# ynotstartups/implisolid

Measured on AMD Instinct MI355X. Metric: Mvoxels/s (eval+MC) at 256^3 & 512^3, higher is better.
Workload: dtype f32; 1 GPU; config4: seeded ~20-node MP5 CSG tree with twist/union/difference (scenes.config4, seed 20251015), box [-1,1]^3, R=512, eval+MC, mesh resident in HBM; resolution=512, voxels=134217728, samples=135005697, cells=135796744, verts=360248, faces=720496, program_instr=42, tree_depth=8, parallelism=zslab1, voxels_per_rank=134217728

## Files before the change

### implisolid_amd/csrc/mc.hip

```cpp
#include <algorithm>
#include <cstdlib>
#include <stdexcept>

#include "eval_bricks.hpp"
#include "ifunc_device.hpp"
#include "kernels.hpp"
#include "mc_device.hpp"
#include "batch_device.hpp"

namespace impli {

GridDesc make_grid(int R, const float box[6], int cz0, int cz1, int cz_emit) {
    GridDesc g{};
    g.R = R;
    g.res = R + 5;
    g.n = R + 3;
    g.m = R + 2;
    for (int a = 0; a < 3; ++a) {
        const float width = box[2 * a + 1] - box[2 * a];
        g.w[a] = width / (float)R;
        g.lo[a] = box[2 * a];
        g.i0[a] = box[2 * a] / g.w[a] - 2.f;
    }
    g.cz0 = cz0;
    g.cz1 = cz1;
    g.cz_emit = cz_emit;
    g.fz0 = cz0;
    g.fz1 = cz1 + 1;
    g.n_cells = (int64_t)g.m * g.m * (cz1 - cz0);
    return g;
}

void build_case_table(CaseInfo out[256]) {
    for (int ci = 0; ci < 256; ++ci) {
        CaseInfo c{};
        const char* s = IMPLI_MC_TRI_CASES[ci];
        int n = 0;
        for (; s[n]; ++n) c.tri[n] = (uint8_t)((s[n] <= '9') ? s[n] - '0' : s[n] - 'a' + 10);
        c.ntri = (uint8_t)(n / 3);
        c.rank[0] = c.rank[1] = c.rank[2] = -1;
        int r = 0;
        for (int k = 0; k < n; ++k) {
            const int e = c.tri[k];
            const int slot = (e == 5) ? 0 : (e == 6) ? 1 : (e == 10) ? 2 : -1;
            if (slot >= 0 && c.rank[slot] < 0) c.rank[slot] = (int8_t)r++;
        }
        c.nown = (uint8_t)r;
        static const int owner_of_edge[12] = {5, 4, 4, 6, 2, 0, 0, 1, 3, 2, 0, 1};
        for (int k = 0; k < n; ++k) c.owners = (uint8_t)(c.owners | (1u << owner_of_edge[c.tri[k]]));
        auto neg = [ci](int k) { return (ci >> k) & 1; };
        const int crossing = (neg(5) ^ neg(6)) + (neg(6) ^ neg(7)) + (neg(2) ^ neg(6));
        int ec = 0, ei = 0, v = 0, ff = 0, opp = 0;
        for (const auto& e : kCubeEdges) { ec += neg(e[0]) ^ neg(e[1]); ei += neg(e[0]) & neg(e[1]); }
        for (int k = 0; k < 8; ++k) v += neg(k);
        for (const auto& f : kCubeFaces) ff += neg(f[0]) & neg(f[1]) & neg(f[2]) & neg(f[3]);
        for (const auto& o : kCubeOpposite) opp += (v == 6 && !neg(o[0]) && !neg(o[1])) ? 1 : 0;
        const int ntri_formula = (ci == 0 || ci == 255) ? 0 : ec - 2 * (v - ei + ff + 2 * opp);
        if (crossing != c.nown || (c.ntri > 0) != (ci != 0 && ci != 255) || ntri_formula != c.ntri)
            throw std::runtime_error("marching cubes: case table violates the count kernel's assumptions");
        out[ci] = c;
    }
}

namespace {

__device__ __forceinline__ uint32_t wave_sum(uint32_t x) {
#pragma unroll
    for (int o = 32; o > 0; o >>= 1) x += __shfl_xor(x, o, 64);
    return x;
}

template <int BS>
__device__ __forceinline__ void mc_count_body(const GridDesc& g, const MCBuffers& b) {
    static_assert(BS % 64 == 0 && BS >= kGroupUnits, "whole waves; wave 0 takes a lane per unit of the group");
    __shared__ uint32_t s_u[kGroupUnits][4];
    __shared__ uint32_t s_cm[kGroupUnits];
    __shared__ uint16_t s_fp[kGroupUnits * kMaxChunks];
    __shared__ uint32_t s_nf;
    const int t = threadIdx.x;
    const int64_t G = blockIdx.x;
    const int nch = n_chunks(g), npairs = kGroupUnits * nch;
    const int64_t rows = n_rows(g), nu = n_units(g);
    const int64_t row0 = G * kGroupUnits * kUnitRows;
    int ui[2], ch[2];
    bool in[2];
    uint32_t mk[2];
    auto marks = [&](int p0) {
#pragma unroll
        for (int q = 0; q < 2; ++q) {
            const int p = p0 + q * BS + t;
            ui[q] = p / nch;
            ch[q] = p - ui[q] * nch;
            in[q] = p < npairs && G * kGroupUnits + ui[q] < nu;
            mk[q] = b.mark_id;
        }
        if (b.umark) {
#pragma unroll
            for (int q = 0; q < 2; ++q) mk[q] = b.umark[in[q] ? (G * kGroupUnits + ui[q]) * nch + ch[q] : 0];
        }
    };
    marks(0);
    for (int k = t; k < 4 * kGroupUnits; k += BS) (&s_u[0][0])[k] = 0u;
    for (int k = t; k < kGroupUnits; k += BS) s_cm[k] = 0u;
    if (t == 0) s_nf = 0u;
    __syncthreads();
    for (int p0 = 0;;) {
        const bool c0 = in[0] & (mk[0] == b.mark_id), c1 = in[1] & (mk[1] == b.mark_id);
        const uint64_t m0 = __ballot(c0), m1 = __ballot(c1);
        const uint32_t n0 = (uint32_t)__popcll((unsigned long long)m0), n1 = (uint32_t)__popcll((unsigned long long)m1);
        const uint64_t below = (1ull << (t & 63)) - 1ull;
        uint32_t base = 0;
        if ((t & 63) == 0 && n0 + n1) base = atomicAdd(&s_nf, n0 + n1);
        base = __shfl(base, 0, 64);
        if (c0) s_fp[base + __popcll((unsigned long long)(m0 & below))] = (uint16_t)(ui[0] * kMaxChunks + ch[0]);
        if (c1) s_fp[base + n0 + __popcll((unsigned long long)(m1 & below))] = (uint16_t)(ui[1] * kMaxChunks + ch[1]);
        p0 += 2 * BS;
        if (p0 >= npairs) break;
        marks(p0);
    }
    __syncthreads();
    const int n_items = (int)s_nf * kUnitRows;
    for (int i = t; i < n_items; i += BS) {
        ChunkBits k;
        const uint32_t pr = s_fp[i / kUnitRows];
        const int ui = (int)(pr / kMaxChunks), c = (int)(pr % kMaxChunks);
        const int rb = ui * kUnitRows + i % kUnitRows;
        const bool ok = row0 + rb < rows;
        load_chunk(g, b.signs, ok ? row0 + rb : 0, c, k);
        if (!ok) k.nt = 0;
        if (!k.nt) continue;
        if (c < kChunkMaskBits) atomicOr(&s_cm[ui], 1u << c);
        const unsigned own = (unsigned)(__popcll((unsigned long long)((k.t01 ^ k.t11) & k.nt)) +
                                        __popcll((unsigned long long)((k.s11 ^ k.t11) & k.nt)) +
                                        __popcll((unsigned long long)((k.t10 ^ k.t11) & k.nt)));
        unsigned tri = 0, act = 0, hal = 0;
        if (k.z >= g.cz_emit) {
            act = (unsigned)__popcll((unsigned long long)k.nt);
            tri = chunk_triangles(k);
        } else {
            hal = own;
        }
        uint32_t* d = s_u[ui];
        if (own) atomicAdd(&d[0], own);
        if (tri) atomicAdd(&d[1], tri);
        atomicAdd(&d[2], act | ((uint32_t)__popcll((unsigned long long)k.nt) << 16));
        if (hal) atomicAdd(&d[3], hal);
    }
    __syncthreads();
    if (t < 64) {
        const int64_t u = G * kGroupUnits + t;
        const uint32_t own = s_u[t][0], tri = s_u[t][1], act = s_u[t][2] & 0xffffu, ntc = s_u[t][2] >> 16, hal = s_u[t][3];
        const bool ne = u < nu && (own | tri) != 0;
        const uint32_t eo = wave_incl_scan<uint32_t>(own, t) - own;
        const uint32_t et = wave_incl_scan<uint32_t>(tri, t) - tri;
        const uint32_t ea = wave_incl_scan<uint32_t>(act, t) - act;
        const uint64_t m = __ballot(ne);
        const uint32_t pos = (uint32_t)__popcll((unsigned long long)(m & ((1ull << t) - 1ull)));
        const uint32_t parts = ne ? min((uint32_t)kMaxParts, max(1u, (act + kPartCells - 1) / kPartCells)) : 0u;
        const bool heavy = act > kHeavyCells;
        const bool small = ne && ntc <= kPairCells && nch <= kChunkMaskBits &&
                           (uint32_t)(kUnitRows * __popc(s_cm[t])) <= kPairCells;
        const uint32_t ph = heavy ? parts : 0u, pl = (heavy || small) ? 0u : parts, ps = small ? 1u : 0u;
        const uint32_t eph = wave_incl_scan<uint32_t>(ph, t) - ph, epl = wave_incl_scan<uint32_t>(pl, t) - pl;
        const uint64_t msm = __ballot(small);
        const uint32_t eps = (uint32_t)__popcll((unsigned long long)(msm & ((1ull << t) - 1ull)));
        if (ne) {
            b.unit_cnt[G * kGroupUnits + pos] = make_uint4((uint32_t)t, eo, et, ea);
            b.unit_part[G * kGroupUnits + pos] =
                (heavy ? eph : small ? eps : epl) | (parts << 16) | ((uint32_t)heavy << 20) | (ps << 21);
            b.unit_cmask[G * kGroupUnits + pos] = s_cm[t];
        }
        const uint32_t sums[kScanParts + 1] = {__shfl(eo + own, 63, 64), __shfl(et + tri, 63, 64),
                                               __shfl(ea + act, 63, 64), wave_sum(hal), __shfl(eph + ph, 63, 64),
                                               __shfl(epl + pl, 63, 64), (uint32_t)__popcll((unsigned long long)msm),
                                               (uint32_t)__popcll((unsigned long long)m)};
        if (t <= kScanParts) {
            const uint32_t v = t == 0 ? sums[0] : t == 1 ? sums[1] : t == 2 ? sums[2] : t == 3 ? sums[3]
                             : t == 4 ? sums[4] : t == 5 ? sums[5] : t == 6 ? sums[6] : sums[7];
            b.scan_blk[(int64_t)t * gridDim.x + G] = v;
        }
    }
}
__global__ __launch_bounds__(512) void k_mc_count(GridDesc g, MCBuffers b) { mc_count_body<512>(g, b); }
__global__ __launch_bounds__(256) void k_mc_count_s(GridDesc g, MCBuffers b) { mc_count_body<256>(g, b); }

constexpr int kScanBlock = 256;
constexpr int kScanRows = kScanParts + 1;
template <int BS = kScanBlock>
__device__ __forceinline__ void unit_scan_body(const GridDesc& g, const MCBuffers& b) {
    static_assert(BS >= kGroupUnits, "a lane per unit of the group");
    __shared__ uint32_t s_part[BS / 64][kScanRows];
    __shared__ uint32_t s_base[kScanRows];
    const int64_t G = blockIdx.x, ng = n_groups(g);
    const int t = threadIdx.x, lane = t & 63, wid = t >> 6;
    const bool last = G == ng - 1;
    const uint32_t nne = b.scan_blk[kScanParts * ng + G];
    if (nne == 0 && !last) return;
    const uint4 e = b.unit_cnt[G * kGroupUnits + (t < (int)nne ? t : 0)];
    const uint32_t pp = b.unit_part[G * kGroupUnits + (t < (int)nne ? t : 0)];
    const uint32_t cm = b.unit_cmask[G * kGroupUnits + (t < (int)nne ? t : 0)];
    uint32_t acc[kScanRows] = {0u, 0u, 0u, 0u, 0u, 0u, 0u, 0u};
#pragma unroll 4
    for (int64_t i = t; i < G; i += BS)
#pragma unroll
        for (int c = 0; c < kScanRows; ++c) acc[c] += b.scan_blk[c * ng + i];
#pragma unroll
    for (int c = 0; c < kScanRows; ++c) {
        const uint32_t s = wave_sum(acc[c]);
        if (lane == 0) s_part[wid][c] = s;
    }
    __syncthreads();
    if (t < kScanRows) {
        uint32_t s = 0;
#pragma unroll
        for (int w = 0; w < BS / 64; ++w) s += s_part[w][t];
        s_base[t] = s;
    }
    __syncthreads();
    if (t < (int)nne) {
        const uint4 ent = make_uint4((uint32_t)(G * kGroupUnits) + e.x, s_base[0] + e.y, s_base[1] + e.z, s_base[2] + e.w);
        const uint32_t P = (pp >> 16) & 15u;
        const bool heavy = (pp >> 20) & 1u, small = (pp >> 21) & 1u;
        const uint32_t r = (heavy ? s_base[4] : small ? s_base[6] : s_base[5]) + (pp & 0xffffu);
        for (uint32_t q = 0; q < P; ++q) {
            const uint32_t at = heavy ? r + q : b.cap_parts - (small ? 2u : 1u) - 2u * (r + q);
            b.ulist[at] = ent;
            b.upart[at] = q | (P << 4) | (cm << 8);
        }
    }
    if (last && t == 0) {
        const uint32_t nh = s_base[4] + b.scan_blk[4 * ng + G];
        const uint32_t ns = s_base[6] + b.scan_blk[6 * ng + G];
        b.counters[7] = nh;
        b.counters[8] = ns;
        b.counters[0] = nh + (ns + 1u) / 2u + s_base[5] + b.scan_blk[5 * ng + G];
        b.counters[1] = s_base[3] + b.scan_blk[3 * ng + G];
        b.counters[2] = s_base[0] + b.scan_blk[G];
        b.counters[3] = s_base[1] + b.scan_blk[ng + G];
        b.counters[4] = s_base[2] + b.scan_blk[2 * ng + G];
        b.counters[5] = s_base[3] + b.scan_blk[3 * ng + G];
        b.counters[6] = s_base[7] + nne;
    }
}
__global__ __launch_bounds__(kScanBlock) void k_unit_scan(GridDesc g, MCBuffers b) { unit_scan_body<>(g, b); }

__global__ __launch_bounds__(64 * kVertsWaves) __attribute__((amdgpu_waves_per_eu(6))) void k_mc_cells(const CaseInfo* __restrict__ cases, GridDesc g, MCBuffers b) {
    mc_cells_body(cases, g, b);
}

constexpr unsigned kFacesBlocks = 2048;
static_assert(kFacesBlocks % 8 == 0, "k_mc_faces' XCD remap needs a multiple of 8 blocks");

__constant__ uint8_t c_edge_owner_idx[12] = {5, 4, 4, 6, 2, 0, 0, 1, 3, 2, 0, 1};
__constant__ uint8_t c_edge_slot[12] = {1, 0, 1, 0, 1, 0, 1, 0, 2, 2, 2, 2};

__device__ __forceinline__ void face_record(const CaseInfo* s_case, uint32_t (*s_w)[256], const GridDesc& g,
                                            const MCBuffers& b, uint32_t Voff, uint32_t i) {
    const int t = threadIdx.x;
    const uint4 r = b.records[i];
    const uint32_t L = r.x, ci = r.y, fbase = r.z;
    const CaseInfo& C = s_case[ci];
    const int ntri = C.ntri;
    if (fbase + ntri > (uint64_t)b.cap_f) { *b.overflow = 1u; return; }
    const uint32_t need = C.owners;
    const uint32_t m = (uint32_t)g.m, m2 = m * m;
    const uint32_t d[6] = {1u, m, m + 1u, m2, m2 + m, m2 + 1u};
    const IdTriple* vid = reinterpret_cast<const IdTriple*>(b.vid);
    IdTriple w[7];
    w[0] = vid[L];
#pragma unroll
    for (int q = 0; q < 6; ++q) w[q + 1] = vid[((need >> (q + 1)) & 1u) ? L - d[q] : L];
#pragma unroll
    for (int e = 0; e < 12; ++e) {
        const IdTriple& q = w[c_edge_owner_idx[e]];
        const int sl = c_edge_slot[e];
        s_w[e][t] = sl == 0 ? q.a : sl == 1 ? q.b : q.c;
    }
    int32_t* out = b.faces + 3 * (size_t)fbase;
    for (int k = 0; k < ntri; ++k) {
        IdTriple f;
        f.a = Voff + s_w[C.tri[3 * k]][t];
        f.b = Voff + s_w[C.tri[3 * k + 1]][t];
        f.c = Voff + s_w[C.tri[3 * k + 2]][t];
        *reinterpret_cast<IdTriple*>(out + 3 * k) = f;
    }
}

__device__ __forceinline__ void mc_faces_body(const CaseInfo* __restrict__ cases, const GridDesc& g, const MCBuffers& b) {
    __shared__ CaseInfo s_case[256];
    __shared__ uint32_t s_w[12][256];
    const int t = threadIdx.x;
    s_case[t] = cases[t];
    __syncthreads();
    const uint32_t n_rec = b.counters[4];
    const uint32_t lim = n_rec < (uint64_t)b.cap_rec ? n_rec : (uint32_t)b.cap_rec;
    uint32_t Voff = b.offsets ? b.offsets[0] : 0u;
    if (b.gathered)
        for (int r = 0; r < b.rank; ++r) Voff += b.gathered[4 * r] - b.gathered[4 * r + 3];
    const uint32_t nb = gridDim.x, lb = (blockIdx.x % 8u) * (nb / 8u) + blockIdx.x / 8u;
    const uint32_t per = (lim + nb - 1u) / nb, i_end = min(lim, (lb + 1u) * per);
    for (uint32_t i = lb * per + t; i < i_end; i += 256) face_record(s_case, s_w, g, b, Voff, i);
}

__global__ __launch_bounds__(256) void k_mc_faces(const CaseInfo* __restrict__ cases, GridDesc g, MCBuffers b) {
    mc_faces_body(cases, g, b);
}

constexpr int kBatchCountLanes = 128;
__global__ __launch_bounds__(kBatchCountLanes) void k_mc_count_b(const ObjArgs* __restrict__ objs, GridDesc g) {
    mc_count_body<kBatchCountLanes>(g, objs[blockIdx.y].mc);
}
template <int B>
__global__ __launch_bounds__(B) void k_unit_scan_b(const ObjArgs* __restrict__ objs, GridDesc g) {
    unit_scan_body<B>(g, objs[blockIdx.y].mc);
}
__global__ __launch_bounds__(64 * kVertsWaves) void k_mc_cells_b(const CaseInfo* __restrict__ cases,
                                                                const ObjArgs* __restrict__ objs, int n, GridDesc g) {
    __shared__ uint32_t s_cw[256];
    __shared__ uint64_t s_bits[kVertsWaves][9][64];
    __shared__ uint32_t s_excl[kVertsWaves][64];
    __shared__ uint32_t s_pre[kMaxBatchObjects + 4];
    const int t = threadIdx.x, wid = t >> 6;
    for (int k = t; k < 256; k += blockDim.x) s_cw[k] = case_word(cases[k]);
    const uint32_t total = batch_prefix(objs, n, 0, 1u, 0xffffffffu, s_pre);
    for (uint32_t e = blockIdx.x * kVertsWaves + wid; e < total; e += gridDim.x * kVertsWaves) {
        const int k = __builtin_amdgcn_readfirstlane(batch_object_of(s_pre, n, e));
        mc_cells_item(s_cw, g, objs[k].mc, e - s_pre[k], s_bits[wid], s_excl[wid]);
    }
}
__global__ __launch_bounds__(256) void k_gather_counters(const ObjArgs* __restrict__ objs, int n, uint32_t* __restrict__ out) {
    const int i = blockIdx.x * 256 + threadIdx.x;
    if (i < n * kCounterWords) out[i] = objs[i / kCounterWords].counters[i % kCounterWords];
}
__global__ __launch_bounds__(256) void k_zero_pieces(const ZeroPiece* __restrict__ pieces) {
    const ZeroPiece z = pieces[blockIdx.x];
    uint8_t* p = reinterpret_cast<uint8_t*>(z.p);
    const uint32_t n16 = z.n / 16;
    for (uint32_t i = threadIdx.x; i < n16; i += 256) reinterpret_cast<uint4*>(p)[i] = uint4{0, 0, 0, 0};
    for (uint32_t i = n16 * 16 + threadIdx.x; i < z.n; i += 256) p[i] = 0;
}
__global__ __launch_bounds__(256) void k_mc_faces_b(const CaseInfo* __restrict__ cases, const ObjArgs* __restrict__ objs,
                                                    int n, GridDesc g) {
    __shared__ CaseInfo s_case[256];
    __shared__ uint32_t s_w[12][256];
    __shared__ uint32_t s_pre[kMaxBatchObjects + 4];
    const int t = threadIdx.x;
    s_case[t] = cases[t];
    const uint32_t total = batch_prefix(objs, n, 4, 1u, 0xffffffffu, s_pre);
    for (uint32_t gi = blockIdx.x * 256 + t; gi < total; gi += gridDim.x * 256) {
        const int k = batch_object_of(s_pre, n, gi);
        const MCBuffers& b = objs[k].mc;
        const uint32_t i = gi - s_pre[k];
        if (i >= (uint64_t)b.cap_rec) { *b.overflow = 1u; continue; }
        face_record(s_case, s_w, g, b, b.offsets ? b.offsets[0] : 0u, i);
    }
}

}

void launch_mc_count(const CaseInfo* d_cases, const GridDesc& g, const MCBuffers& b, hipStream_t s) {
    const int64_t ng = n_groups(g);
    if (ng == 0) return;
    (void)d_cases;
    if (n_chunks(g) == 1) k_mc_count_s<<<(unsigned)ng, 256, 0, s>>>(g, b);
    else k_mc_count<<<(unsigned)ng, 512, 0, s>>>(g, b);
}

void launch_mc_scan(const GridDesc& g, const MCBuffers& b, hipStream_t s) {
    const int64_t ng = n_groups(g);
    if (ng > 0) k_unit_scan<<<(unsigned)ng, kScanBlock, 0, s>>>(g, b);
}

void launch_mc_faces(const CaseInfo* d_cases, const GridDesc& g, const MCBuffers& b, hipStream_t s) {
    k_mc_faces<<<kFacesBlocks, 256, 0, s>>>(d_cases, g, b);
}

void launch_mc_verts(const CaseInfo* d_cases, const GridDesc& g, const MCBuffers& b, hipStream_t s) {
    const int64_t nu = n_units(g);
    if (nu > 0) {
        k_mc_cells<<<(unsigned)std::min<int64_t>((nu + kVertsWaves - 1) / kVertsWaves, kVertsMaxBlocks),
                     64 * kVertsWaves, 0, s>>>(d_cases, g, b);
    }
}

}

namespace impli {

constexpr unsigned kBatchCellBlocks = 4096, kBatchFaceBlocks = 2048;

void launch_gather_counters(const ObjArgs* d_objs, int n, uint32_t* d_out, hipStream_t s) {
    if (n > 0) k_gather_counters<<<(unsigned)((n * kCounterWords + 255) / 256), 256, 0, s>>>(d_objs, n, d_out);
}

void launch_zero_pieces(const ZeroPiece* d_pieces, int n, hipStream_t s) {
    if (n > 0) k_zero_pieces<<<(unsigned)n, 256, 0, s>>>(d_pieces);
}

void launch_batch_mc(const ObjArgs* d_objs, int n, const CaseInfo* d_cases, const GridDesc& g, hipStream_t s) {
    const int64_t ng = n_groups(g), nu = n_units(g);
    if (ng == 0 || n <= 0) return;
    k_mc_count_b<<<dim3((unsigned)ng, (unsigned)n), kBatchCountLanes, 0, s>>>(d_objs, g);
    if (ng <= 64) k_unit_scan_b<64><<<dim3((unsigned)ng, (unsigned)n), 64, 0, s>>>(d_objs, g);
    else k_unit_scan_b<kScanBlock><<<dim3((unsigned)ng, (unsigned)n), kScanBlock, 0, s>>>(d_objs, g);
    (void)nu;
    k_mc_cells_b<<<kBatchCellBlocks, 64 * kVertsWaves, 0, s>>>(d_cases, d_objs, n, g);
    k_mc_faces_b<<<kBatchFaceBlocks, 256, 0, s>>>(d_cases, d_objs, n, g);
}

}
```

Measured before the change: 1.438 million Mvoxels/s.

## Batch scan loads with DPP reductions and pack face case tables into shared memory

The unit scan kernel now issues several iterations of scan_blk loads before accumulating, replaces the shuffle-based wave sum with a DPP row reduction plus readlane, drops one block barrier and the s_base stage, and reads the group's own sums through lanes 0-7. The faces kernel packs each case's triangle edge indices into a 64-bit nibble word and its owners/ntri into one word in shared memory, and prefetches the next record before each face_record call. The scan kernels also get a waves-per-EU hint. The aim is to cut latency in the scan and shared-memory traffic in the faces kernel, at the cost of more code complexity and possible register pressure.

```diff
diff --git a/implisolid_amd/csrc/mc.hip b/implisolid_amd/csrc/mc.hip
--- a/implisolid_amd/csrc/mc.hip
+++ b/implisolid_amd/csrc/mc.hip
@@ -186,63 +186,92 @@
 
 constexpr int kScanBlock = 256;
 constexpr int kScanRows = kScanParts + 1;
+constexpr int kScanAhead = 4;
+__device__ __forceinline__ uint32_t wave_total_dpp(uint32_t x) {
+    x += (uint32_t)__builtin_amdgcn_update_dpp(0, (int)x, 0x111, 0xf, 0xf, false);
+    x += (uint32_t)__builtin_amdgcn_update_dpp(0, (int)x, 0x112, 0xf, 0xf, false);
+    x += (uint32_t)__builtin_amdgcn_update_dpp(0, (int)x, 0x114, 0xf, 0xf, false);
+    x += (uint32_t)__builtin_amdgcn_update_dpp(0, (int)x, 0x118, 0xf, 0xf, false);
+    x += (uint32_t)__builtin_amdgcn_update_dpp(0, (int)x, 0x142, 0xa, 0xf, false);
+    x += (uint32_t)__builtin_amdgcn_update_dpp(0, (int)x, 0x143, 0xc, 0xf, false);
+    return (uint32_t)__builtin_amdgcn_readlane((int)x, 63);
+}
+__device__ __forceinline__ uint32_t load_at(const uint32_t* p, uint32_t i) {
+    return *reinterpret_cast<const uint32_t*>(reinterpret_cast<const char*>(p) + (i << 2));
+}
 template <int BS = kScanBlock>
 __device__ __forceinline__ void unit_scan_body(const GridDesc& g, const MCBuffers& b) {
-    static_assert(BS >= kGroupUnits, "a lane per unit of the group");
-    __shared__ uint32_t s_part[BS / 64][kScanRows];
-    __shared__ uint32_t s_base[kScanRows];
-    const int64_t G = blockIdx.x, ng = n_groups(g);
-    const int t = threadIdx.x, lane = t & 63, wid = t >> 6;
-    const bool last = G == ng - 1;
-    const uint32_t nne = b.scan_blk[kScanParts * ng + G];
-    if (nne == 0 && !last) return;
-    const uint4 e = b.unit_cnt[G * kGroupUnits + (t < (int)nne ? t : 0)];
-    const uint32_t pp = b.unit_part[G * kGroupUnits + (t < (int)nne ? t : 0)];
-    const uint32_t cm = b.unit_cmask[G * kGroupUnits + (t < (int)nne ? t : 0)];
+    static_assert(BS >= kGroupUnits && BS % 64 == 0, "a lane per unit of the group, whole waves");
+    static_assert(kScanRows == 8, "lanes 0-7 of a wave hold the group's own sums");
+    constexpr int W = BS / 64;
+    __shared__ uint32_t s_part[kScanRows][W];
+    const uint32_t G = blockIdx.x, ng = (uint32_t)n_groups(g);
+    const uint32_t t = threadIdx.x, lane = t & 63u, wid = t >> 6;
+    const bool last = G == ng - 1u;
+    const uint32_t mine = b.scan_blk[(lane & 7u) * ng + G];
+    const uint32_t slot = G * kGroupUnits + (t & (uint32_t)(kGroupUnits - 1));
+    const uint4 e = b.unit_cnt[slot];
+    const uint32_t pp = b.unit_part[slot];
+    const uint32_t cm = b.unit_cmask[slot];
     uint32_t acc[kScanRows] = {0u, 0u, 0u, 0u, 0u, 0u, 0u, 0u};
-#pragma unroll 4
-    for (int64_t i = t; i < G; i += BS)
-#pragma unroll
-        for (int c = 0; c < kScanRows; ++c) acc[c] += b.scan_blk[c * ng + i];
-#pragma unroll
-    for (int c = 0; c < kScanRows; ++c) {
-        const uint32_t s = wave_sum(acc[c]);
-        if (lane == 0) s_part[wid][c] = s;
-    }
+    for (uint32_t i0 = 0; i0 < G; i0 += kScanAhead * BS) {
+        uint32_t v[kScanAhead][kScanRows];
+#pragma unroll
+        for (int q = 0; q < kScanAhead; ++q) {
+            const uint32_t i = i0 + q * BS + t;
+#pragma unroll
+            for (int c = 0; c < kScanRows; ++c) v[q][c] = load_at(b.scan_blk + c * ng, i < G ? i : 0u);
+        }
+#pragma unroll
+        for (int q = 0; q < kScanAhead; ++q)
+#pragma unroll
+            for (int c = 0; c < kScanRows; ++c) acc[c] += i0 + q * BS + t < G ? v[q][c] : 0u;
+    }
+    uint32_t tot[kScanRows];
+#pragma unroll
+    for (int c = 0; c < kScanRows; ++c) tot[c] = wave_total_dpp(acc[c]);
+    if (lane == 0) {
+#pragma unroll
+        for (int c = 0; c < kScanRows; ++c) s_part[c][wid] = tot[c];
+    }
+    const uint32_t nne = (uint32_t)__builtin_amdgcn_readlane((int)mine, kScanParts);
     __syncthreads();
-    if (t < kScanRows) {
+    auto base = [&](int c) {
         uint32_t s = 0;
 #pragma unroll
-        for (int w = 0; w < BS / 64; ++w) s += s_part[w][t];
-        s_base[t] = s;
-    }
-    __syncthreads();
-    if (t < (int)nne) {
-        const uint4 ent = make_uint4((uint32_t)(G * kGroupUnits) + e.x, s_base[0] + e.y, s_base[1] + e.z, s_base[2] + e.w);
+        for (int w = 0; w < W; ++w) s += s_part[c][w];
+        return s;
+    };
+    if (t < nne) {
+        const uint4 ent = make_uint4(G * kGroupUnits + e.x, base(0) + e.y, base(1) + e.z, base(2) + e.w);
         const uint32_t P = (pp >> 16) & 15u;
         const bool heavy = (pp >> 20) & 1u, small = (pp >> 21) & 1u;
-        const uint32_t r = (heavy ? s_base[4] : small ? s_base[6] : s_base[5]) + (pp & 0xffffu);
+        const uint32_t r = base(heavy ? 4 : small ? 6 : 5) + (pp & 0xffffu);
         for (uint32_t q = 0; q < P; ++q) {
             const uint32_t at = heavy ? r + q : b.cap_parts - (small ? 2u : 1u) - 2u * (r + q);
             b.ulist[at] = ent;
             b.upart[at] = q | (P << 4) | (cm << 8);
         }
     }
-    if (last && t == 0) {
-        const uint32_t nh = s_base[4] + b.scan_blk[4 * ng + G];
-        const uint32_t ns = s_base[6] + b.scan_blk[6 * ng + G];
-        b.counters[7] = nh;
-        b.counters[8] = ns;
-        b.counters[0] = nh + (ns + 1u) / 2u + s_base[5] + b.scan_blk[5 * ng + G];
-        b.counters[1] = s_base[3] + b.scan_blk[3 * ng + G];
-        b.counters[2] = s_base[0] + b.scan_blk[G];
-        b.counters[3] = s_base[1] + b.scan_blk[ng + G];
-        b.counters[4] = s_base[2] + b.scan_blk[2 * ng + G];
-        b.counters[5] = s_base[3] + b.scan_blk[3 * ng + G];
-        b.counters[6] = s_base[7] + nne;
-    }
-}
-__global__ __launch_bounds__(kScanBlock) void k_unit_scan(GridDesc g, MCBuffers b) { unit_scan_body<>(g, b); }
+    if (last && t < 64u) {
+        const uint32_t total = base((int)(lane & 7u)) + mine;
+        uint32_t T[kScanRows];
+#pragma unroll
+        for (int c = 0; c < kScanRows; ++c) T[c] = (uint32_t)__builtin_amdgcn_readlane((int)total, c);
+        if (t == 0) {
+            b.counters[7] = T[4];
+            b.counters[8] = T[6];
+            b.counters[0] = T[4] + (T[6] + 1u) / 2u + T[5];
+            b.counters[1] = T[3];
+            b.counters[2] = T[0];
+            b.counters[3] = T[1];
+            b.counters[4] = T[2];
+            b.counters[5] = T[3];
+            b.counters[6] = T[7];
+        }
+    }
+}
+__global__ __launch_bounds__(kScanBlock) __attribute__((amdgpu_waves_per_eu(8))) void k_unit_scan(GridDesc g, MCBuffers b) { unit_scan_body<>(g, b); }
 
 __global__ __launch_bounds__(64 * kVertsWaves) __attribute__((amdgpu_waves_per_eu(6))) void k_mc_cells(const CaseInfo* __restrict__ cases, GridDesc g, MCBuffers b) {
     mc_cells_body(cases, g, b);
@@ -254,15 +283,26 @@
 __constant__ uint8_t c_edge_owner_idx[12] = {5, 4, 4, 6, 2, 0, 0, 1, 3, 2, 0, 1};
 __constant__ uint8_t c_edge_slot[12] = {1, 0, 1, 0, 1, 0, 1, 0, 2, 2, 2, 2};
 
-__device__ __forceinline__ void face_record(const CaseInfo* s_case, uint32_t (*s_w)[256], const GridDesc& g,
-                                            const MCBuffers& b, uint32_t Voff, uint32_t i) {
+struct FaceCases {
+    uint64_t tri[256];
+    uint32_t ow[256];
+};
+__device__ __forceinline__ void face_case_store(FaceCases& fc, int ci, const CaseInfo& c) {
+    uint64_t tri = 0;
+#pragma unroll
+    for (int k = 0; k < 15; ++k) tri |= (uint64_t)(c.tri[k] & 15u) << (4 * k);
+    fc.tri[ci] = tri;
+    fc.ow[ci] = (uint32_t)c.owners | ((uint32_t)c.ntri << 8);
+}
+__device__ __forceinline__ void face_record(const FaceCases& fc, uint32_t (*s_w)[256], const GridDesc& g,
+                                            const MCBuffers& b, uint32_t Voff, const uint4 r) {
     const int t = threadIdx.x;
-    const uint4 r = b.records[i];
     const uint32_t L = r.x, ci = r.y, fbase = r.z;
-    const CaseInfo& C = s_case[ci];
-    const int ntri = C.ntri;
+    const uint32_t ow = fc.ow[ci];
+    uint64_t tri = fc.tri[ci];
+    const int ntri = (int)(ow >> 8);
     if (fbase + ntri > (uint64_t)b.cap_f) { *b.overflow = 1u; return; }
-    const uint32_t need = C.owners;
+    const uint32_t need = ow & 0xffu;
     const uint32_t m = (uint32_t)g.m, m2 = m * m;
     const uint32_t d[6] = {1u, m, m + 1u, m2, m2 + m, m2 + 1u};
     const IdTriple* vid = reinterpret_cast<const IdTriple*>(b.vid);
@@ -277,29 +317,37 @@
         s_w[e][t] = sl == 0 ? q.a : sl == 1 ? q.b : q.c;
     }
     int32_t* out = b.faces + 3 * (size_t)fbase;
-    for (int k = 0; k < ntri; ++k) {
+    for (int k = 0; k < ntri; ++k, tri >>= 12) {
         IdTriple f;
-        f.a = Voff + s_w[C.tri[3 * k]][t];
-        f.b = Voff + s_w[C.tri[3 * k + 1]][t];
-        f.c = Voff + s_w[C.tri[3 * k + 2]][t];
+        f.a = Voff + s_w[(uint32_t)tri & 15u][t];
+        f.b = Voff + s_w[((uint32_t)tri >> 4) & 15u][t];
+        f.c = Voff + s_w[((uint32_t)tri >> 8) & 15u][t];
         *reinterpret_cast<IdTriple*>(out + 3 * k) = f;
     }
 }
 
 __device__ __forceinline__ void mc_faces_body(const CaseInfo* __restrict__ cases, const GridDesc& g, const MCBuffers& b) {
-    __shared__ CaseInfo s_case[256];
+    __shared__ FaceCases s_fc;
     __shared__ uint32_t s_w[12][256];
     const int t = threadIdx.x;
-    s_case[t] = cases[t];
-    __syncthreads();
+    const CaseInfo c = cases[t];
     const uint32_t n_rec = b.counters[4];
-    const uint32_t lim = n_rec < (uint64_t)b.cap_rec ? n_rec : (uint32_t)b.cap_rec;
     uint32_t Voff = b.offsets ? b.offsets[0] : 0u;
     if (b.gathered)
         for (int r = 0; r < b.rank; ++r) Voff += b.gathered[4 * r] - b.gathered[4 * r + 3];
+    const uint32_t lim = n_rec < (uint64_t)b.cap_rec ? n_rec : (uint32_t)b.cap_rec;
     const uint32_t nb = gridDim.x, lb = (blockIdx.x % 8u) * (nb / 8u) + blockIdx.x / 8u;
     const uint32_t per = (lim + nb - 1u) / nb, i_end = min(lim, (lb + 1u) * per);
-    for (uint32_t i = lb * per + t; i < i_end; i += 256) face_record(s_case, s_w, g, b, Voff, i);
+    const uint32_t first = lb * per;
+    uint32_t i = first + t;
+    uint4 r = *(first < i_end ? b.records + (i < i_end ? i : first) : reinterpret_cast<const uint4*>(cases));
+    face_case_store(s_fc, t, c);
+    __syncthreads();
+    while (i < i_end) {
+        face_record(s_fc, s_w, g, b, Voff, r);
+        i += 256;
+        if (i < i_end) r = b.records[i];
+    }
 }
 
 __global__ __launch_bounds__(256) void k_mc_faces(const CaseInfo* __restrict__ cases, GridDesc g, MCBuffers b) {
@@ -311,7 +359,7 @@
     mc_count_body<kBatchCountLanes>(g, objs[blockIdx.y].mc);
 }
 template <int B>
-__global__ __launch_bounds__(B) void k_unit_scan_b(const ObjArgs* __restrict__ objs, GridDesc g) {
+__global__ __launch_bounds__(B) __attribute__((amdgpu_waves_per_eu(8))) void k_unit_scan_b(const ObjArgs* __restrict__ objs, GridDesc g) {
     unit_scan_body<B>(g, objs[blockIdx.y].mc);
 }
 __global__ __launch_bounds__(64 * kVertsWaves) void k_mc_cells_b(const CaseInfo* __restrict__ cases,
@@ -341,18 +389,18 @@
 }
 __global__ __launch_bounds__(256) void k_mc_faces_b(const CaseInfo* __restrict__ cases, const ObjArgs* __restrict__ objs,
                                                     int n, GridDesc g) {
-    __shared__ CaseInfo s_case[256];
+    __shared__ FaceCases s_fc;
     __shared__ uint32_t s_w[12][256];
     __shared__ uint32_t s_pre[kMaxBatchObjects + 4];
     const int t = threadIdx.x;
-    s_case[t] = cases[t];
+    face_case_store(s_fc, t, cases[t]);
     const uint32_t total = batch_prefix(objs, n, 4, 1u, 0xffffffffu, s_pre);
     for (uint32_t gi = blockIdx.x * 256 + t; gi < total; gi += gridDim.x * 256) {
         const int k = batch_object_of(s_pre, n, gi);
         const MCBuffers& b = objs[k].mc;
         const uint32_t i = gi - s_pre[k];
         if (i >= (uint64_t)b.cap_rec) { *b.overflow = 1u; continue; }
-        face_record(s_case, s_w, g, b, b.offsets ? b.offsets[0] : 0u, i);
+        face_record(s_fc, s_w, g, b, b.offsets ? b.offsets[0] : 0u, b.records[i]);
     }
 }
 
```

Measured after the change: 1.480 million Mvoxels/s, median of 6. 1.03x the previous value.
